# Amanda-Zheng/MR-GNAS

Hardware: AMD Instinct MI355X
Metric: million edges/sec per supernet fwd+bwd step (FB15k-237, dim=200) (higher is better)
Workload: dtype f32

## Files before the change

include/mrgnas.h:

```cpp
#ifndef MRGNAS_H
#define MRGNAS_H

#include <stdint.h>

#ifdef __cplusplus
extern "C" {
#endif

#define MRG_ABI_VERSION 21

#define MRG_OK            0
#define MRG_E_NULLPTR    -1
#define MRG_E_SHAPE      -2
#define MRG_E_ENUM       -3
#define MRG_E_WORKSPACE  -4

#define MRG_COMPOSE_MULT 0
#define MRG_COMPOSE_SUB  1
#define MRG_COMPOSE_ADD  2
#define MRG_REDUCE_SUM   0
#define MRG_REDUCE_MEAN  1
#define MRG_REDUCE_MAX   2
#define MRG_GCS_SUB      0
#define MRG_GCS_MUL      1
#define MRG_GCS_COPY     2
#define MRG_GCS_NEGS     3
#define MRG_GCS_CCORR    4
#define MRG_GCS_CCONV    5
#define MRG_ACT_NONE     0
#define MRG_ACT_RELU     1
#define MRG_ACT_SIGMOID  2

int mrg_abi_version(void);
const char *mrg_error_string(int code);
const char *mrg_target_arch(void);

int mrg_compose_fwd(int op, const float *s, const float *hr, float *out,
                    int64_t rows, int D, void *stream);
int mrg_compose_bwd(int op, const float *gout, const float *s, const float *hr,
                    float *gs, float *ghr, int64_t rows, int D, void *stream);

int mrg_gather_compose_fwd(int op, const float *ent, const float *rel,
                           const int32_t *ent_idx, const int32_t *rel_idx,
                           float *out, int64_t rows, int D, void *stream);

#define MRG_GATE_LD(D) (2 * (D) + 4)

int mrg_gate_collapse3(const float *const *W_host, const float *const *b_host, const float *const *a_host, float *uvc,
                       int D, int in_dim, int fold, void *stream);
int mrg_gate_param_grad3(const float *const *W_host, const float *const *b_host, const float *const *a_host,
                         const float *d_uvc, float *const *gW_host, float *const *gb_host, float *const *ga_host,
                         int D, int in_dim, int fold, void *stream);
int mrg_fold_halves3(const float *const *W_host, float *Wt, int D, void *stream);
int mrg_unfold_halves3(const float *const *gWt_host, float *const *gW_host, int D, void *stream);

int mrg_gate_fwd(const float *s, const float *s_in, const float *norm, const float *uvc,
                 float *out, int64_t b0, int64_t b1, int64_t M, int D, float scale, void *stream);
int64_t mrg_gate_bwd_workspace_bytes(int64_t M, int D);
int mrg_gate_bwd(const float *gout, const float *s, const float *s_in, const float *norm,
                 const float *uvc, float *gs, float *gs_in, float *d_uvc, void *ws,
                 int64_t b0, int64_t b1, int64_t M, int D, float scale, void *stream);
int mrg_gate_row_fwd(const float *s, const float *s_in, const float *norm, const float *uvc, float *fvec, float *hvec,
                     int64_t b0, int64_t b1, int64_t M, int D, float scale, void *stream);
int64_t mrg_gate_row_colsum_blocks(int64_t b0, int64_t b1, int64_t M, int D, int vec4);
int mrg_gate_row_fwd_colsum(const float *s, const float *s_in, const float *norm, const float *uvc, float *fvec, float *hvec,
                            int64_t b0, int64_t b1, int64_t M, int D, float scale, void *stream, double *colsum, int64_t colsum_blocks);
int mrg_gate_row_bwd(const float *q, const float *hvec, const float *s, const float *s_in, const float *uvc, float *gs_in, float *d_uvc,
                     void *ws, int64_t b0, int64_t b1, int64_t M, int D, void *stream);

int64_t mrg_seg_reduce_workspace_bytes(int64_t n_slots, int D);
int mrg_seg_reduce_fwd(int mode, const float *msg, const float *self_rows,
                       const int32_t *eid,
                       const int32_t *chunk_node, const int32_t *chunk_start, const int32_t *chunk_end,
                       const int32_t *chunk_slot, int64_t n_chunks,
                       const int32_t *hub_node, const int32_t *hub_first, const int32_t *hub_count, int64_t n_hubs,
                       int64_t n_slots, const int32_t *in_degree,
                       float *out, int32_t *arg, void *ws,
                       int64_t N, int D, void *stream);
int mrg_seg_reduce_bwd(int mode, const float *gout, const int32_t *dst, const int32_t *in_degree,
                       const int32_t *arg, float *gmsg, float *gself, const float *relu_src,
                       int64_t E, int64_t N, int D, void *stream);
int mrg_seg_reduce_bwd_ordered(int mode, const float *gout, const int32_t *dst, const int32_t *in_degree, const int32_t *arg,
                               float *gmsg, float *gself, const float *relu_src, const unsigned *relu_bits, const int32_t *order,
                               int64_t E, int64_t N, int D, void *stream);
int mrg_segmax_bwd_input_ok(int D, int Kin);
int mrg_segmax_bwd_input(const float *gout, const float *mx, const int32_t *dst, const int32_t *arg, const float *W, float *gmsg,
                         float *gx, const int32_t *order, int64_t E, int64_t N, int D, int Kin, void *stream);

int64_t mrg_seg_std_workspace_bytes(int64_t n_slots, int D);
int mrg_seg_std_fwd(const float *msg, const int32_t *eid, const int32_t *chunk_node, const int32_t *chunk_start,
                    const int32_t *chunk_end, const int32_t *chunk_slot, int64_t n_chunks, const int32_t *hub_node,
                    const int32_t *hub_first, const int32_t *hub_count, int64_t n_hubs, int64_t n_slots,
                    const int32_t *in_degree, float *out, float *mean, float *coef, void *ws, int64_t N, int D, void *stream);
int mrg_seg_std_bwd(const float *gout, const float *msg, const int32_t *dst, const float *mean, const float *coef,
                    const int32_t *order, float *gmsg, int64_t E, int64_t N, int D, void *stream);

int mrg_fused_gcs(int mode, const float *X, const int32_t *xi, const float *Y, const int32_t *yi,
                  const float *scal, const int32_t *eid,
                  const int32_t *chunk_node, const int32_t *chunk_start, const int32_t *chunk_end,
                  const int32_t *chunk_slot, int64_t n_chunks,
                  const int32_t *hub_node, const int32_t *hub_first, const int32_t *hub_count, int64_t n_hubs,
                  int64_t n_slots, const int32_t *seg_len,
                  float *out, void *ws, int64_t nseg, int D, void *stream);

int mrg_span_gcs(int mode, const float *X, const float *Y, const void *meta, const float *ext_scal, int64_t E, int span,
                 const int32_t *span_slot, const int32_t *span_start, int64_t n_spans,
                 const int32_t *hub_seg, const int32_t *hub_first, const int32_t *hub_count, int64_t n_hubs,
                 int64_t n_slots, const int32_t *seg_len,
                 float *out, void *ws, int64_t nseg, int D, void *stream);

int mrg_sum_buffers(const float *const *xs_host, int K, float *out, int64_t n, int accumulate, void *stream);
int mrg_sum_rows_gather(const float *const *xs_host, int K, const float *gather_edge, const float *gather_self,
                        const int32_t *dst, int64_t E, int64_t rows, int D, float *out, void *stream);

int mrg_distmult_score(const float *ent, const float *rel, const int32_t *s_idx, const int32_t *r_idx,
                       const int32_t *o_idx, float *score, int64_t T, int D, void *stream);

int64_t mrg_mix_workspace_bytes(int K, int D);

int mrg_optim_chunk(void);
int mrg_clip_sgd_step(void *const *params, const void *const *grads, void *const *bufs, const int32_t *chunk_tensor,
                      const int64_t *chunk_off, const int32_t *chunk_len, int64_t n_chunks, double *partial, float *norm_coef,
                      float max_norm, float lr, float momentum, float weight_decay, void *stream);
int mrg_adam_step(void *const *params, const void *const *grads, void *const *exp_avg, void *const *exp_avg_sq, int64_t n_tensors,
                  const int32_t *chunk_tensor, const int64_t *chunk_off, const int32_t *chunk_len, int64_t n_chunks, float *step,
                  float *scal, const float *lr, double beta1, double beta2, float eps, float weight_decay, void *stream);
#define MRG_MIX_MAX_CANDIDATES 8
typedef struct mrg_gated_branch {
  int32_t k;
  const float *s;
  const float *rowscale;
  int32_t row_k;
  const float *row_f;
  const float *row_h;
  const float *row_uvc;
  int32_t row_ld;
  int64_t b0, b1;
  float *row_dq;
  int32_t act;
  const int32_t *valid_rows;
// ... 181 lines not shown
```

mr-gnas_amd/_lib.py:

```python
import ctypes
import os
import re

import torch

_HERE = os.path.dirname(os.path.abspath(__file__))
LIB_PATH = os.environ.get("MRG_LIB_PATH") or os.path.join(_HERE, "lib", "libmrgnas_hip.so")
HEADER_PATH = os.path.join(os.path.dirname(_HERE), "include", "mrgnas.h")

ABI_VERSION = 21


class MrgnasLibraryError(RuntimeError):
    pass


class MrgnasError(RuntimeError):
    """A C-ABI call returned a non-zero code."""


_P, _I, _L, _F = ctypes.c_void_p, ctypes.c_int, ctypes.c_int64, ctypes.c_float

SIGNATURES = {
    "mrg_abi_version": (_I, []),
    "mrg_error_string": (ctypes.c_char_p, [_I]),
    "mrg_target_arch": (ctypes.c_char_p, []),
    "mrg_compose_fwd": (_I, [_I, _P, _P, _P, _L, _I, _P]),
    "mrg_compose_bwd": (_I, [_I, _P, _P, _P, _P, _P, _L, _I, _P]),
    "mrg_gather_compose_fwd": (_I, [_I, _P, _P, _P, _P, _P, _L, _I, _P]),
    "mrg_gate_collapse3": (_I, [_P, _P, _P, _P, _I, _I, _I, _P]),
    "mrg_gate_param_grad3": (_I, [_P, _P, _P, _P, _P, _P, _P, _I, _I, _I, _P]),
    "mrg_fold_halves3": (_I, [_P, _P, _I, _P]),
    "mrg_unfold_halves3": (_I, [_P, _P, _I, _P]),
    "mrg_gate_fwd": (_I, [_P, _P, _P, _P, _P, _L, _L, _L, _I, _F, _P]),
    "mrg_gate_bwd_workspace_bytes": (_L, [_L, _I]),
    "mrg_gate_bwd": (_I, [_P, _P, _P, _P, _P, _P, _P, _P, _P, _L, _L, _L, _I, _F, _P]),
    "mrg_seg_reduce_workspace_bytes": (_L, [_L, _I]),
    "mrg_seg_reduce_fwd": (_I, [_I, _P, _P, _P, _P, _P, _P, _P, _L, _P, _P, _P, _L, _L, _P, _P, _P, _P, _L, _I, _P]),
    "mrg_seg_reduce_bwd": (_I, [_I, _P, _P, _P, _P, _P, _P, _P, _L, _L, _I, _P]),
    "mrg_fused_gcs": (_I, [_I, _P, _P, _P, _P, _P, _P, _P, _P, _P, _P, _L, _P, _P, _P, _L, _L, _P, _P, _P, _L, _I, _P]),
    "mrg_span_gcs": (_I, [_I, _P, _P, _P, _P, _L, _I, _P, _P, _L, _P, _P, _P, _L, _L, _P, _P, _P, _L, _I, _P]),
    "mrg_sum_buffers": (_I, [_P, _I, _P, _L, _I, _P]),
    "mrg_sum_rows_gather": (_I, [_P, _I, _P, _P, _P, _L, _L, _I, _P, _P]),
    "mrg_distmult_score": (_I, [_P, _P, _P, _P, _P, _P, _L, _I, _P]),
    "mrg_gate_row_fwd": (_I, [_P, _P, _P, _P, _P, _P, _L, _L, _L, _I, _F, _P]),
    "mrg_gate_row_colsum_blocks": (_L, [_L, _L, _L, _I, _I]),
    "mrg_gate_row_fwd_colsum": (_I, [_P, _P, _P, _P, _P, _P, _L, _L, _L, _I, _F, _P, _P, _L]),
    "mrg_gate_row_bwd": (_I, [_P, _P, _P, _P, _P, _P, _P, _P, _L, _L, _L, _I, _P]),
    "mrg_mix_workspace_bytes": (_L, [_I, _I]),
    "mrg_mix_colstats": (_I, [_P, _I, _L, _I, _P, _P, _P, _P]),
    "mrg_mix_finalize_fwd": (_I, [_P, _P, _P, _P, _P, _I, ctypes.c_double, _I, _F, _F, _P, _P]),
    "mrg_mix_stats_coef": (_I, [_P, _P, _P, _P, _P, _I, _L, ctypes.c_double, _I, _F, _F, _P, _P, _P, _P]),
    "mrg_zero_workspace_bytes": (_L, [_I]),
    "mrg_zero_colstats": (_I, [_P, _P, _P, _P, _P, _I, _L, _I, _P, _P, _P]),
    "mrg_zero_stats_coef": (_I, [_P, _P, _P, _P, _P, _I, _P, _P, _P, _P, _L, ctypes.c_double, _I, _F, _F, _P, _P, _P, _P]),
    "mrg_zero_fwd": (_I, [_P, _P, _P, _P, _P, _I, _P, _P, _P, _L, _I, _P, _P]),
    "mrg_zero_bwd_reduce": (_I, [_P, _P, _P, _P, _P, _P, _I, _P, _P, _P, _P, _L, _I, _P, _P]),
    "mrg_zero_bwd_apply": (_I, [_P, _P, _P, _P, _P, _P, _I, _P, _P, _P, _P, _P, _L, _I, _P, _P]),
    "mrg_mix_fwd": (_I, [_P, _I, _P, _P, _P, _P, _L, _I, _P, _P]),
    "mrg_mix_bwd_reduce": (_I, [_P, _P, _I, _P, _P, _P, _P, _L, _I, _P, _P]),
    "mrg_mix_finalize_bwd": (_I, [_P, _I, ctypes.c_double, _I, _P, _P, _P, _P, _P, _P]),
    "mrg_mix_bwd_apply": (_I, [_P, _P, _P, _I, _P, _P, _P, _P, _P, _P, _P, _P, _P, _P, _P, _P, _P, _L, _I, _P, _P]),
    "mrg_dense_filter_fwd": (_I, [_I, _P, _P, _P, _P, _P, _F, _P, _P, _P, _L, _I, _P]),
    "mrg_dense_filter_dz": (_I, [_I, _P, _P, _P, _P, _F, _P, _P, _L, _I, _P]),
    "mrg_gemm_workspace_bytes": (_L, [_I, _I]),
    "mrg_gemm_set_mode": (_I, [_I]),
    "mrg_gemm_set_epilogue": (_I, [_I]),
    "mrg_gemm_set_wide8": (_I, [_I]),
    "mrg_gemm_set_q": (_I, [_I]),
    "mrg_gemm_set_small": (_I, [_I]),
    "mrg_segmax_bwd_input_ok": (_I, [_I, _I]),
    "mrg_segmax_bwd_input": (_I, [_P, _P, _P, _P, _P, _P, _P, _P, _L, _L, _I, _I, _P]),
    "mrg_seg_std_workspace_bytes": (_L, [_L, _I]),
    "mrg_seg_std_fwd": (_I, [_P, _P, _P, _P, _P, _P, _L, _P, _P, _P, _L, _L, _P, _P, _P, _P, _P, _L, _I, _P]),
    "mrg_seg_std_bwd": (_I, [_P, _P, _P, _P, _P, _P, _P, _L, _L, _I, _P]),
    "mrg_optim_chunk": (_I, []),
    "mrg_clip_sgd_step": (_I, [_P, _P, _P, _P, _P, _P, _L, _P, _P, _F, _F, _F, _F, _P]),
    "mrg_adam_step": (_I, [_P, _P, _P, _P, _L, _P, _P, _P, _L, _P, _P, _P, ctypes.c_double, ctypes.c_double, _F, _F, _P]),
    "mrg_act_grad_transpose": (_I, [_P, _P, _P, _L, _L, _I, _P]),
    "mrg_wgrad_set_variant": (_I, [_I]),
    "mrg_linear_fwd": (_I, [_P, _P, _P, _P, _P, _L, _I, _I, _I, _P]),
    "mrg_dense_filter3_workspace_bytes": (_L, [_I, _I]),
    "mrg_dense_filter_fwd3": (_I, [_I, _P, _P, _P, _P, _P, _F, _F, _P, _P, _P, _L, _L, _L, _I, _P]),
    "mrg_dense_filter3_colsum_blocks": (_L, [_I, _L, _L, _L, _I, _I]),
    "mrg_dense_filter_fwd3_colsum": (_I, [_I, _P, _P, _P, _P, _P, _F, _F, _P, _P, _P, _L, _L, _L, _I, _P, _P, _L]),
    "mrg_dense_filter_dz3": (_I, [_I, _P, _P, _P, _P, _F, _F, _P, _P, _L, _L, _I, _P]),
    "mrg_linear_bwd_input3_workspace_bytes": (_L, [_I, _I]),
    "mrg_linear_bwd_input3": (_I, [_P, _P, _P, _P, _L, _L, _L, _I, _I, _I, _I, _P]),
    "mrg_linear_bwd_input3_pair_workspace_bytes": (_L, [_I, _I]),
    "mrg_linear_bwd_input3_pair": (_I, [_P, _P, _P, _P, _P, _P, _L, _L, _L, _I, _I, _I, _I, _P]),
    "mrg_linear_bwd_weight3_workspace_bytes": (_L, [_L, _L, _L, _I, _I, _I]),
    "mrg_linear_bwd_weight3": (_I, [_P, _P, _P, _P, _P, _P, _L, _L, _L, _I, _I, _I, _P]),
    "mrg_linear_relu_segsum_fwd": (_I, [_P, _P, _P, _P, _P, _P, _P, _P, _L, _I, _I, _P]),
    "mrg_seg_reduce_heads_fwd": (_I, [_I, _P, _P, _P, _P, _P, _P, _P, _L, _P, _P, _P, _L, _L, _P, _P, _P, _L, _I, _P]),
    "mrg_seg_reduce_bwd_bits": (_I, [_I, _P, _P, _P, _P, _P, _P, _L, _L, _I, _P]),
    "mrg_seg_reduce_bwd_ordered": (_I, [_I, _P, _P, _P, _P, _P, _P, _P, _P, _P, _L, _L, _I, _P]),
    "mrg_linear_relu_segmax_workspace_bytes": (_L, [_L, _I, _I]),
    "mrg_linear_relu_segmax_fwd": (_I, [_P, _P, _P, _P, _P, _P, _P, _P, _P, _P, _L, _L, _I, _I, _P]),
    "mrg_linear_bwd_input_workspace_bytes": (_L, [_I, _I]),
    "mrg_linear_bwd_input": (_I, [_P, _P, _P, _P, _L, _I, _I, _I, _I, _P]),
    "mrg_linear_bwd_weight_workspace_bytes": (_L, [_L, _I, _I]),
    "mrg_linear_bwd_weight": (_I, [_P, _P, _P, _P, _P, _P, _L, _I, _I, _I, _P]),
    "mrg_linear_bwd_weight_share": (_I, [_P, _P, _P, _P, _P, _P, _L, _I, _I, _I, _I, _P]),
    "mrg_build_graph_workspace_bytes": (_L, [_L]),
    "mrg_build_graph": (_I, [_P, _L, _L, _I, _I, _P, _L, _P, _P, _P, _P, _P, _P, _P, _P, _P, _P, _L, _P]),
    "mrg_plan_workspace_bytes": (_L, [_L, _L, _I]),
    "mrg_span_plan_build": (_I, [_P, _L, _L, _I, _I, _P, _P, _P, _P, _P, _P, _P, _P, _P, _P, _L, _P]),
    "mrg_span_meta_pack": (_I, [_P, _P, _P, _P, _P, _I, _P, _L, _P]),
    "mrg_chunk_plan_workspace_bytes": (_L, [_L, _L]),
    "mrg_chunk_plan_build": (_I, [_P, _L, _L, _I, _P, _P, _P, _P, _P, _P, _P, _P, _P, _P, _P, _P, _L, _P]),
    "mrg_negative_sampling": (_I, [_P, _L, _I, _P, _P, _P, _P, _P]),
    "mrg_sample_neighborhood_workspace_bytes": (_L, [_L, _L]),
    "mrg_sample_edge_neighborhood": (_I, [_P, _P, _P, _P, _L, _L, _L, _P, _P, _L, _P, _P, _P, _P, _L, _P]),
    "mrg_relabel_workspace_bytes": (_L, [_L]),
    "mrg_relabel_nodes": (_I, [_P, _P, _L, _L, _P, _P, _P, _P, _P, _L, _P]),
    "mrg_multi_hot_labels": (_I, [_P, _P, _P, _P, _L, _L, _L, _F, _F, _P, _P]),
    "mrg_rank_filtered": (_I, [_P, _P, _P, _L, _L, _P, _P]),
    "mrg_transe_score_fwd": (_I, [_P, _P, _P, _F, _P, _L, _L, _I, _P]),
    "mrg_transe_score_bwd": (_I, [_P, _P, _P, _P, _P, _P, _P, _L, _L, _I, _P]),
    "mrg_ccorr_rows": (_I, [_I, _P, _P, _P, _L, _I, _P]),
    "mrg_ccorr_matrix": (_I, [_I, _P, _P, _I, _P]),
    "mrg_ccorr_matrix_grad": (_I, [_I, _P, _P, _I, _P]),
    "mrg_conve_fc_workspace_bytes": (_L, [_L, _L, _I]),
    "mrg_conve_bwd_workspace_bytes": (_L, [_L, _I, _I, _I]),
    "mrg_conve_bn0_fwd": (_I, [_P, _P, _L, _I, _P, _P, _I, _F, _F, _P, _P]),
# ... 178 lines not shown
```

mr-gnas_amd/csrc/segreduce.hip:

```cpp
#include "segcommon.hpp"

namespace mrg {

__device__ __forceinline__ bool seg_is_head(int j, int list_start) {
  const int q = j & 31;
  const int prev = (q & 3) ? j - 1 : (q >= 8 ? j - 5 : -1);
  return prev < list_start;
}

template <int VEC, int LPR, int KMAX, bool IS_MAX, bool HEADS = false>
__global__ __launch_bounds__(MRG_BLOCK) void seg_chunk_k(const float* __restrict__ msg, const float* __restrict__ self_rows,
                                                         const int32_t* __restrict__ eid, const int32_t* __restrict__ chunk_node,
                                                         const int32_t* __restrict__ chunk_start, const int32_t* __restrict__ chunk_end,
                                                         const int32_t* __restrict__ chunk_slot, int64_t n_chunks,
                                                         const int32_t* __restrict__ in_degree, float* __restrict__ out,
                                                         int32_t* __restrict__ arg, float* __restrict__ ws_val,
                                                         int32_t* __restrict__ ws_arg, int D, int is_mean,
                                                         const int32_t* __restrict__ head_rowptr = nullptr) {
  constexpr int RPB = MRG_BLOCK / LPR;
  constexpr int U = 4;
  const int sl = threadIdx.x % LPR, rw = row_group_of_thread<LPR>();
  const int dv = D / VEC;
  for (int64_t ch = (int64_t)blockIdx.x * RPB + rw; ch < n_chunks; ch += (int64_t)gridDim.x * RPB) {
    const int v = chunk_node[ch];
// ... 108 lines not shown
  const int dv = D >> 2, kv = Kin >> 2;
  const int64_t stride = (int64_t)gridDim.x * WAVES;
  auto edge_at = [&](int64_t p) -> int { const int64_t q = p < E ? p : E - 1; return order ? order[q] : (int)q; };
  const bool lv = lane < dv;
  auto load_row = [&](int64_t v, float4& g4, int4& a4, float4& x4) {
    g4 = make_float4(0.f, 0.f, 0.f, 0.f); a4 = make_int4(-1, -1, -1, -1); x4 = make_float4(1.f, 1.f, 1.f, 1.f);
    if (lv) {
      g4 = *reinterpret_cast<const float4*>(gout + v * D + lane * 4);
      a4 = *reinterpret_cast<const int4*>(arg + v * D + lane * 4);
      if (mx) x4 = *reinterpret_cast<const float4*>(mx + v * D + lane * 4);
    }
  };
  const int64_t first = (int64_t)blockIdx.x * WAVES + wave;
  if (first >= E) return;
  int r0 = __builtin_amdgcn_readfirstlane(edge_at(first));
  int r1 = __builtin_amdgcn_readfirstlane(edge_at(first + stride));
  int64_t v1 = __builtin_amdgcn_readfirstlane(dst[r1]);
  float4 g4, x4; int4 a4;
  load_row((int64_t)__builtin_amdgcn_readfirstlane(dst[r0]), g4, a4, x4);
  for (int64_t pos = first; pos < E; pos += stride) {
    const int r2 = __builtin_amdgcn_readfirstlane(edge_at(pos + 2 * stride));
    const int v2 = dst[r2];
    float4 gn, xn; int4 an;
    load_row(v1, gn, an, xn);
    const int r = r0;
    float m[4];
    m[0] = (a4.x == r && x4.x > 0.f) ? g4.x : 0.f;
    m[1] = (a4.y == r && x4.y > 0.f) ? g4.y : 0.f;
    m[2] = (a4.z == r && x4.z > 0.f) ? g4.z : 0.f;
    m[3] = (a4.w == r && x4.w > 0.f) ? g4.w : 0.f;
    if (lv && gmsg) *reinterpret_cast<float4*>(gmsg + (int64_t)r * D + lane * 4) = make_float4(m[0], m[1], m[2], m[3]);
    float4 acc = make_float4(0.f, 0.f, 0.f, 0.f);
#pragma unroll
    for (int j = 0; j < 4; ++j) {
      unsigned long long live = __ballot(m[j] != 0.f);
      while (live) {
        const int src = __builtin_amdgcn_readfirstlane((int)__builtin_ctzll(live));
        live &= live - 1;
        const float val = __int_as_float(__builtin_amdgcn_readlane(__float_as_int(m[j]), src));
        const int c = src * 4 + j;
        if (lane < kv) {
          const float4 w4 = *reinterpret_cast<const float4*>(wsrc + c * Kin + lane * 4);
          acc.x += val * w4.x; acc.y += val * w4.y; acc.z += val * w4.z; acc.w += val * w4.w;
        }
      }
    }
    if (lane < kv) *reinterpret_cast<float4*>(gx + (int64_t)r * Kin + lane * 4) = acc;
    g4 = gn; a4 = an; x4 = xn;
    r0 = r1; r1 = r2;
    v1 = __builtin_amdgcn_readfirstlane(v2);
  }
}

}

using namespace mrg;

extern "C" int mrg_segmax_bwd_input_ok(int D, int Kin) {
  return (D > 0 && Kin > 0 && D % 4 == 0 && Kin % 4 == 0 && D <= 256 && Kin <= 256 && (size_t)D * Kin * 4 <= 160 * 1024) ? 1 : 0;
}

extern "C" int mrg_segmax_bwd_input(const float* gout, const float* mx, const int32_t* dst, const int32_t* arg, const float* W, float* gmsg,
                                    float* gx, const int32_t* order, int64_t E, int64_t N, int D, int Kin, void* stream) {
  if (E < 0 || N < 0 || E >= ((int64_t)1 << 31)) return MRG_E_SHAPE;
  if (!mrg_segmax_bwd_input_ok(D, Kin)) return MRG_E_SHAPE;
  if (E == 0) return MRG_OK;
  if (!gout || !dst || !arg || !W || !gx) return MRG_E_NULLPTR;
  if (!aligned16(gout) || !aligned16(arg) || !aligned16(W) || !aligned16(gx) || !aligned16(gmsg) || !aligned16(mx)) return MRG_E_SHAPE;
  const size_t lds = (size_t)D * Kin * sizeof(float);
  (void)hipFuncSetAttribute(reinterpret_cast<const void*>(&segmax_bwd_gx_k), hipFuncAttributeMaxDynamicSharedMemorySize, (int)lds);
  int64_t grid = (E + 15) / 16;
  if (grid > 256) grid = 256;
  hipLaunchKernelGGL(segmax_bwd_gx_k, dim3((unsigned)grid), dim3(1024), lds, (hipStream_t)stream, gout, mx, dst, arg, W, gmsg, gx, order, E, D, Kin);
  MRG_LAUNCH_CHECK();
  return MRG_OK;
}

extern "C" int64_t mrg_seg_reduce_workspace_bytes(int64_t n_slots, int D) {
  if (n_slots < 0 || D <= 0) return 0;
  return (n_slots + 1) * (int64_t)D * 8 + 64;
}

static int seg_reduce_fwd_impl(int mode, const float* msg, const float* self_rows, const int32_t* eid,
                               const int32_t* chunk_node, const int32_t* chunk_start, const int32_t* chunk_end,
                               const int32_t* chunk_slot, int64_t n_chunks, const int32_t* hub_node,
                               const int32_t* hub_first, const int32_t* hub_count, int64_t n_hubs, int64_t n_slots,
                               const int32_t* in_degree, float* out, int32_t* arg, void* ws, int64_t N, int D,
                               void* stream, const int32_t* head_rowptr);

extern "C" int mrg_seg_reduce_fwd(int mode, const float* msg, const float* self_rows, const int32_t* eid,
                                  const int32_t* chunk_node, const int32_t* chunk_start, const int32_t* chunk_end,
                                  const int32_t* chunk_slot, int64_t n_chunks, const int32_t* hub_node,
                                  const int32_t* hub_first, const int32_t* hub_count, int64_t n_hubs, int64_t n_slots,
                                  const int32_t* in_degree, float* out, int32_t* arg, void* ws, int64_t N, int D,
                                  void* stream) {
  return seg_reduce_fwd_impl(mode, msg, self_rows, eid, chunk_node, chunk_start, chunk_end, chunk_slot, n_chunks, hub_node, hub_first,
                             hub_count, n_hubs, n_slots, in_degree, out, arg, ws, N, D, stream, nullptr);
}

extern "C" int mrg_seg_reduce_heads_fwd(int mode, const float* part, const float* self_rows, const int32_t* rowptr,
                                        const int32_t* chunk_node, const int32_t* chunk_start, const int32_t* chunk_end,
                                        const int32_t* chunk_slot, int64_t n_chunks, const int32_t* hub_node,
                                        const int32_t* hub_first, const int32_t* hub_count, int64_t n_hubs, int64_t n_slots,
                                        const int32_t* in_degree, float* out, void* ws, int64_t N, int D, void* stream) {
  if (mode != MRG_REDUCE_SUM && mode != MRG_REDUCE_MEAN) return MRG_E_ENUM;
  if (!rowptr) return MRG_E_NULLPTR;
  return seg_reduce_fwd_impl(mode, part, self_rows, nullptr, chunk_node, chunk_start, chunk_end, chunk_slot, n_chunks, hub_node, hub_first,
                             hub_count, n_hubs, n_slots, in_degree, out, nullptr, ws, N, D, stream, rowptr);
}
// ... 93 lines not shown
```

mr-gnas_amd/functional/reducers.py:

```python
import os

import torch

from .. import _lib
from .._lib import call, f32c, ptr, require_hip, stream_of
from . import switches as SW
from ._base import REDUCE, _cnt, _ws, _ws_bytes
from .gcs import span_gcs


def _seg_fwd(mode, msg, self_rows, p, N, D, want_arg=True):
    out = torch.empty(N, D, dtype=torch.float32, device=msg.device)
    arg = torch.empty(N, D, dtype=torch.int32, device=msg.device) if mode == 2 else None
    n_chunks, n_hubs, n_slots = _cnt(p, "chunks"), _cnt(p, "hubs"), _cnt(p, "slots")
    ws = _ws(_ws_bytes("mrg_seg_reduce_workspace_bytes", n_slots, D), msg) if n_slots > 0 else None
    E = int(p["eid"].numel())
    nb = 4 * D * E + 4 * E + 4 * D * N * (1 + (self_rows is not None) + (mode == 2))
    call("mrg_seg_reduce_fwd", (mode, ptr(msg), ptr(self_rows), ptr(p["eid"]), ptr(p["chunk_node"]), ptr(p["chunk_start"]),
                                ptr(p["chunk_end"]), ptr(p["chunk_slot"]), n_chunks, ptr(p["hub_node"]),
                                ptr(p["hub_first"]), ptr(p["hub_count"]), n_hubs, n_slots, ptr(p["in_degree"]),
                                ptr(out), ptr(arg), ptr(ws), N, D, stream_of(msg)), nbytes=nb)
    return out, arg


ORDERED_BWD = os.environ.get("MRG_SEG_BWD_ORDERED", "1") == "1"
ORDERED_BWD_MIN_BYTES = int(os.environ.get("MRG_SEG_BWD_ORDERED_MIN_BYTES", str(128 << 20)))


def _seg_bwd(mode, g, graph, arg, gmsg, gself, relu_src=None, relu_bits=None):
    p = graph.plan()
    E, N, D = graph.num_edges(), graph.number_of_nodes(), g.shape[1]
    nb = 4 * D * E * (1 + (relu_src is not None)) + 4 * E + 4 * D * N * (1 + (gself is not None) + (mode == 2))
    big = 4 * D * N * (2 if mode == 2 else 1) > ORDERED_BWD_MIN_BYTES
    order = p["eid"] if (ORDERED_BWD and g.is_cuda and big) else None
    call("mrg_seg_reduce_bwd_ordered", (mode, ptr(g), ptr(graph.i32("dst")), ptr(p["in_degree"]), ptr(arg), ptr(gmsg), ptr(gself),
                                        ptr(relu_src), ptr(relu_bits), ptr(order), E, N, D, stream_of(g)), nbytes=nb)



def _amax_bwd_sparse(g, mx, arg, W, graph, gy, gx):
    E, N, D = graph.num_edges(), graph.number_of_nodes(), g.shape[1]
    if not (SW.SPARSE_AMAX_BWD and g.is_cuda and _lib.load().mrg_segmax_bwd_input_ok(D, W.shape[1])):
        return False
    p = graph.plan()
    big = 4 * D * N * 3 > ORDERED_BWD_MIN_BYTES
    order = p["eid"] if (ORDERED_BWD and big) else None
    call("mrg_segmax_bwd_input", (ptr(g), ptr(mx), ptr(graph.i32("dst")), ptr(arg), ptr(W), ptr(gy), ptr(gx), ptr(order), E, N, D, W.shape[1],
                                  stream_of(g)), nbytes=4 * E * (D + W.shape[1]) + 4 * E + 12 * N * D)
    return True

class _SegReduce(torch.autograd.Function):
    @staticmethod
    def forward(ctx, mode, msg, self_rows, graph):
        msg, self_rows = f32c(msg), f32c(self_rows)
        require_hip(msg, self_rows)
        if msg.shape[0] != graph.num_edges():
            raise _lib.MrgnasError(f"message rows {msg.shape[0]} != number of edges {graph.num_edges()}")
        if mode != 2 and hasattr(graph, "agg_plan"):
            sp, meta = graph.agg_plan("mean" if mode == 1 else "sum")
            out, arg = span_gcs("copy", msg, None, meta, sp), None
            if self_rows is not None:
                out += self_rows
        else:
            out, arg = _seg_fwd(mode, msg, self_rows, graph.plan(), graph.number_of_nodes(), msg.shape[1])
        ctx.mode, ctx.graph, ctx.has_self = mode, graph, self_rows is not None
        ctx.save_for_backward(*((arg,) if arg is not None else ()))
        return out

    @staticmethod
    def backward(ctx, g):
        g = f32c(g)
        arg = ctx.saved_tensors[0] if ctx.mode == 2 else None
        gmsg = torch.empty(ctx.graph.num_edges(), g.shape[1], dtype=torch.float32, device=g.device)
        _seg_bwd(ctx.mode, g, ctx.graph, arg, gmsg, None)
        return None, gmsg, (g if ctx.has_self else None), None


def seg_reduce(kind, msg, self_rows, graph):
    return _SegReduce.apply(REDUCE[kind], msg, self_rows, graph)


class _AggRows(torch.autograd.Function):

    @staticmethod
    def forward(ctx, mode, x, graph, add_self, keep):
        x = f32c(x)
        require_hip(x, keep)
        E, N, D = graph.num_edges(), graph.number_of_nodes(), x.shape[1]
        if x.shape[0] != E + N:
            raise _lib.MrgnasError(f"expected {E + N} rows (E + N), got {x.shape[0]}")
        if mode != 2 and hasattr(graph, "agg_plan"):
            sp, meta = graph.agg_plan("mean" if mode == 1 else "sum")
            out, arg = span_gcs("copy", x, None, meta, sp), None
            if keep is not None:
                out *= keep
            if add_self:
                out += x[E:]
        else:
            out, arg = _seg_fwd(mode, x, x[E:] if (add_self and keep is None) else None, graph.plan(), N, D)
            if keep is not None:
                out *= keep
                if add_self:
# ... 59 lines not shown
            ctx.mode, ctx.graph, ctx.fused = mode, graph, True
            ctx.save_for_backward(x, W, arg, mx)
            if SW.MASK_TAP is not None:
                SW.MASK_TAP(("a_max", W.data_ptr()), [arg, mx > 0])
            return out
        if (mode == 1 and SW.FUSED_AMEAN and E >= SW.FUSED_AMAX_MIN_ROWS and hasattr(graph, "plan")
                and _fused_agg_ws(N, D) > 0):
            p = graph.plan()
            part = torch.empty(E, D, dtype=torch.float32, device=x.device)
            bits = torch.empty(E, (D + 31) // 32, dtype=torch.int32, device=x.device)
            gws = _ws(_ws_bytes("mrg_gemm_workspace_bytes", D, D), x)
            call("mrg_linear_relu_segsum_fwd", (ptr(x), ptr(W), ptr(b), ptr(p["eid"]), ptr(graph.i32("dst")), ptr(part), ptr(bits), ptr(gws),
                                                E, D, D, st), nbytes=4 * E * D + 8 * E + 4 * D * D, flops=2 * E * D * D)
            out = torch.empty(N, D, dtype=torch.float32, device=x.device)
            n_chunks, n_hubs, n_slots = _cnt(p, "chunks"), _cnt(p, "hubs"), _cnt(p, "slots")
            ws = _ws(_ws_bytes("mrg_seg_reduce_workspace_bytes", n_slots, D), x) if n_slots > 0 else None
            call("mrg_seg_reduce_heads_fwd", (1, ptr(part), ptr(x[E:]), ptr(p["rowptr"]), ptr(p["chunk_node"]), ptr(p["chunk_start"]),
                                              ptr(p["chunk_end"]), ptr(p["chunk_slot"]), n_chunks, ptr(p["hub_node"]), ptr(p["hub_first"]),
                                              ptr(p["hub_count"]), n_hubs, n_slots, ptr(p["in_degree"]), ptr(out), ptr(ws), N, D, st),
                 nbytes=8 * N * D + 4 * E)
            ctx.mode, ctx.graph, ctx.fused = mode, graph, "mean"
            ctx.save_for_backward(x, W, bits)
            if SW.MASK_TAP is not None:
                SW.MASK_TAP(("a_mean", W.data_ptr()), [bits])
            return out
        y = torch.empty(E, D, dtype=torch.float32, device=x.device)
        gws = _ws(_ws_bytes("mrg_gemm_workspace_bytes", D, D), x)
        call("mrg_linear_fwd", (ptr(x), ptr(W), ptr(b), ptr(y), ptr(gws), E, D, D, 1, st),
             nbytes=4 * E * 2 * D + 4 * D * D, flops=2 * E * D * D)
        if mode == 2:
            out, arg = _seg_fwd(2, y, x[E:], graph.plan(), N, D)
        else:
            sp, meta = graph.agg_plan("mean" if mode == 1 else "sum")
            out, arg = span_gcs("copy", y, None, meta, sp), None
            out += x[E:]
        ctx.mode, ctx.graph, ctx.fused = mode, graph, False
        ctx.save_for_backward(x, W, y, *((arg,) if arg is not None else ()))
        return out

    @staticmethod
    def backward(ctx, g):
        graph, mode = ctx.graph, ctx.mode
        g = f32c(g)
        if ctx.fused == "mean":
            x, W, bits = ctx.saved_tensors
        elif ctx.fused:
            x, W, arg, mx = ctx.saved_tensors
        else:
            x, W, y, *rest = ctx.saved_tensors
            arg = rest[0] if rest else None
        E, N, D = graph.num_edges(), graph.number_of_nodes(), x.shape[1]
        st = stream_of(x)
        gx = torch.empty_like(x)
        gy = torch.empty(E, D, dtype=torch.float32, device=x.device)
        if ctx.fused == "mean":
            _seg_bwd(1, g, graph, None, gy, gx[E:], relu_bits=bits)
        elif ctx.fused:
            gx[E:] = g
            have_gx = _amax_bwd_sparse(g, mx, arg, W, graph, gy, gx)
            if not have_gx:
                _seg_bwd(mode, g * (mx > 0), graph, arg, gy, None)
        else:
            _seg_bwd(mode, g, graph, arg, gy, gx[E:], relu_src=y)
        work = dict(nbytes=4 * E * 2 * D + 4 * D * D, flops=2 * E * D * D)
        if not (ctx.fused is True and have_gx):
            wt = _ws(_ws_bytes("mrg_linear_bwd_input_workspace_bytes", D, D), x)
            call("mrg_linear_bwd_input", (ptr(gy), ptr(W), ptr(gx), ptr(wt), E, D, D, D, 0, st), **work)
        gW = torch.empty_like(W)
        gb = torch.empty(D, dtype=torch.float32, device=x.device)
        ws = _ws(_ws_bytes("mrg_linear_bwd_weight_workspace_bytes", E, D, D), x)
        call("mrg_linear_bwd_weight", (ptr(gy), ptr(x), None, ptr(gW), ptr(gb), ptr(ws), E, D, 0, D, st), **work)
        return None, gx, gW, gb, None


def linear_relu_aggregate(kind, x, W, b, graph):
    return _LinReluAgg.apply(REDUCE[kind], x, W, b, graph)


class _LinReluPartial(torch.autograd.Function):

    @staticmethod
    def forward(ctx, mode, x, W, b, graph):
        x, W, b = f32c(x), f32c(W), f32c(b)
        require_hip(x, W, b)
        E, N, D = graph.num_edges(), graph.number_of_nodes(), x.shape[1]
        st = stream_of(x)
        fused_ws = _fused_agg_ws(N, D) if (mode == 2 and SW.FUSED_AMAX and E >= SW.FUSED_AMAX_MIN_ROWS) else 0
        if fused_ws > 0:
            out = torch.empty(N, D, dtype=torch.float32, device=x.device)
            arg = torch.empty(N, D, dtype=torch.int32, device=x.device)
            mx = torch.empty(N, D, dtype=torch.float32, device=x.device)
            call("mrg_linear_relu_segmax_fwd", (ptr(x), ptr(W), ptr(b), ptr(graph.plan()["eid"]), ptr(graph.i32("dst")), None, ptr(out), ptr(arg),
                                                ptr(mx), ptr(_ws(fused_ws, x)), E, N, D, D, st),
                 nbytes=4 * E * D + 8 * E + 4 * D * D + 4 * N * D * 3, flops=2 * E * D * D)
            ctx.mode, ctx.graph, ctx.fused = mode, graph, True
            ctx.save_for_backward(x, W, arg, mx)
            if SW.MASK_TAP is not None:
                SW.MASK_TAP(("a_max", W.data_ptr()), [arg, mx > 0])
            return out, x[E:].clone()
        if (mode != 2 and SW.FUSED_AMEAN and E >= SW.FUSED_AMAX_MIN_ROWS and _fused_agg_ws(N, D) > 0):
            p = graph.plan()
            part = torch.empty(E, D, dtype=torch.float32, device=x.device)
            bits = torch.empty(E, (D + 31) // 32, dtype=torch.int32, device=x.device)
            gws = _ws(_ws_bytes("mrg_gemm_workspace_bytes", D, D), x)
            call("mrg_linear_relu_segsum_fwd", (ptr(x), ptr(W), ptr(b), ptr(p["eid"]), ptr(graph.i32("dst")), ptr(part), ptr(bits), ptr(gws),
                                                E, D, D, st), nbytes=4 * E * D + 8 * E + 4 * D * D, flops=2 * E * D * D)
            out = torch.empty(N, D, dtype=torch.float32, device=x.device)
            n_chunks, n_hubs, n_slots = _cnt(p, "chunks"), _cnt(p, "hubs"), _cnt(p, "slots")
            ws = _ws(_ws_bytes("mrg_seg_reduce_workspace_bytes", n_slots, D), x) if n_slots > 0 else None
            call("mrg_seg_reduce_heads_fwd", (0, ptr(part), None, ptr(p["rowptr"]), ptr(p["chunk_node"]), ptr(p["chunk_start"]),
                                              ptr(p["chunk_end"]), ptr(p["chunk_slot"]), n_chunks, ptr(p["hub_node"]), ptr(p["hub_first"]),
                                              ptr(p["hub_count"]), n_hubs, n_slots, ptr(p["in_degree"]), ptr(out), ptr(ws), N, D, st),
                 nbytes=8 * N * D + 4 * E)
            ctx.mode, ctx.graph, ctx.fused = mode, graph, "sum"
            ctx.save_for_backward(x, W, bits)
            return out, x[E:].clone()
        y = torch.empty(E, D, dtype=torch.float32, device=x.device)
        gws = _ws(_ws_bytes("mrg_gemm_workspace_bytes", D, D), x)
        call("mrg_linear_fwd", (ptr(x), ptr(W), ptr(b), ptr(y), ptr(gws), E, D, D, 1, st),
             nbytes=4 * E * 2 * D + 4 * D * D, flops=2 * E * D * D)
        if mode == 2:
            out, arg = _seg_fwd(2, y, None, graph.plan(), N, D)
        else:
            sp, meta = graph.agg_plan("sum")
            out, arg = span_gcs("copy", y, None, meta, sp), None
        ctx.mode, ctx.graph, ctx.fused = mode, graph, False
        ctx.save_for_backward(x, W, y, *((arg,) if arg is not None else ()))
        return out, x[E:].clone()

    @staticmethod
    def backward(ctx, g, gself):
        if ctx.fused == "sum":
            x, W, bits = ctx.saved_tensors
        elif ctx.fused:
            x, W, arg, mx = ctx.saved_tensors
        else:
            x, W, y, *rest = ctx.saved_tensors
            arg = rest[0] if rest else None
        graph, mode = ctx.graph, ctx.mode
        E, D = graph.num_edges(), x.shape[1]
        g = f32c(g) if g is not None else torch.zeros(graph.number_of_nodes(), D, dtype=torch.float32, device=x.device)
        st = stream_of(x)
        gx = torch.empty_like(x)
        if gself is not None:
            gx[E:] = gself
        else:
            gx[E:].zero_()
        gy = torch.empty(E, D, dtype=torch.float32, device=x.device)
        if ctx.fused == "sum":
            _seg_bwd(0, g, graph, None, gy, None, relu_bits=bits)
        elif ctx.fused:
            have_gx = _amax_bwd_sparse(g, mx, arg, W, graph, gy, gx)
            if not have_gx:
                _seg_bwd(mode, g * (mx > 0), graph, arg, gy, None)
        else:
            _seg_bwd(mode, g, graph, arg, gy, None, relu_src=y)
        work = dict(nbytes=4 * E * 2 * D + 4 * D * D, flops=2 * E * D * D)
        if not (ctx.fused is True and have_gx):
            wt = _ws(_ws_bytes("mrg_linear_bwd_input_workspace_bytes", D, D), x)
            call("mrg_linear_bwd_input", (ptr(gy), ptr(W), ptr(gx), ptr(wt), E, D, D, D, 0, st), **work)
        gW = torch.empty_like(W)
        gb = torch.empty(D, dtype=torch.float32, device=x.device)
        ws = _ws(_ws_bytes("mrg_linear_bwd_weight_workspace_bytes", E, D, D), x)
        call("mrg_linear_bwd_weight", (ptr(gy), ptr(x), None, ptr(gW), ptr(gb), ptr(ws), E, D, 0, D, st), **work)
        return None, gx, gW, gb, None


def linear_relu_partial(kind, x, W, b, graph):
    return _LinReluPartial.apply(REDUCE[kind], x, W, b, graph)


class _SumPartial(torch.autograd.Function):

    @staticmethod
    def forward(ctx, x, graph):
        x = f32c(x)
        require_hip(x)
        E = graph.num_edges()
        sp, meta = graph.agg_plan("sum")
        ctx.graph = graph
        ctx.shape = x.shape
        return span_gcs("copy", x, None, meta, sp), x[E:].clone()

    @staticmethod
    def backward(ctx, g, gself):
        graph = ctx.graph
        E, D = graph.num_edges(), ctx.shape[1]
        gx = torch.empty(ctx.shape, dtype=torch.float32, device=(g if g is not None else gself).device)
        if gself is not None:
            gx[E:] = gself
        else:
            gx[E:].zero_()
        if g is not None:
            _seg_bwd(0, f32c(g), graph, None, gx, None)
        else:
            gx[:E].zero_()
        return gx, None


def sum_partial(x, graph):
    return _SumPartial.apply(x, graph)
```

mr-gnas_amd/functional/switches.py:

```python
import os

ROW_FACTOR = os.environ.get("MRG_ROW_FACTOR", "1") == "1"
LAZY_ASUM = os.environ.get("MRG_LAZY_ASUM", "1") == "1"
FUSED_AMAX = os.environ.get("MRG_FUSED_AMAX", "1") == "1"
FUSED_AMAX_MIN_ROWS = int(os.environ.get("MRG_FUSED_AMAX_MIN_ROWS", "100000"))
FUSED_AMEAN = os.environ.get("MRG_FUSED_AMEAN", "1") == "1"
WIDE_BWD_INPUT = os.environ.get("MRG_WIDE_BWD_INPUT", "1") == "1"
NODE_LINEAR = os.environ.get("MRG_NODE_LINEAR", "1") == "1"
MASK_TAP = None
FOLD_IDENTITY = os.environ.get("MRG_FOLD_IDENTITY", "1") == "1"
CELL_ZERO_FUSED = os.environ.get("MRG_CELL_ZERO_FUSED", "1") == "1"
FORK_MIN_ROWS = int(os.environ.get("MRG_FORK_MIN_ROWS", str(1 << 17)))
SEGMENT_STREAMS = int(os.environ.get("MRG_SEGMENT_STREAMS", "3"))
FOLD_ROW_SCALE = os.environ.get("MRG_FOLD_ROW_SCALE", "1") == "1"
GROUPED_SEGMENTS = os.environ.get("MRG_GROUPED_SEGMENTS", "1") == "1"
DENSE_PAIR = os.environ.get("MRG_DENSE_PAIR", "1") == "1"
GATED_RECOMPUTE = os.environ.get("MRG_GATED_RECOMPUTE", "1") == "1"
PRODUCER_STATS = os.environ.get("MRG_PRODUCER_STATS", "1") == "1"
COMPGCN_TAIL = os.environ.get("MRG_COMPGCN_TAIL", "1") == "1"
SPARSE_AMAX_BWD = os.environ.get("MRG_SPARSE_AMAX_BWD", "1") == "1"
CCORR_PATH = None
```

Baseline: 11.76.

## Compute max-aggregation weight gradient sparsely from argmax winners, skipping dense gy

```diff
diff --git a/include/mrgnas.h b/include/mrgnas.h
--- a/include/mrgnas.h
+++ b/include/mrgnas.h
@@ -7,7 +7,7 @@
 extern "C" {
 #endif
 
-#define MRG_ABI_VERSION 21
+#define MRG_ABI_VERSION 22
 
 #define MRG_OK            0
 #define MRG_E_NULLPTR    -1
@@ -86,6 +86,10 @@
 int mrg_segmax_bwd_input_ok(int D, int Kin);
 int mrg_segmax_bwd_input(const float *gout, const float *mx, const int32_t *dst, const int32_t *arg, const float *W, float *gmsg,
                          float *gx, const int32_t *order, int64_t E, int64_t N, int D, int Kin, void *stream);
+int mrg_segmax_bwd_weight_ok(int D, int K);
+int64_t mrg_segmax_bwd_weight_workspace_bytes(int64_t E, int D, int K);
+int mrg_segmax_bwd_weight(const float *gout, const float *mx, const int32_t *arg, const float *x, const int32_t *eid,
+                          const int32_t *dst, float *gW, float *gb, void *ws, int64_t E, int64_t N, int D, int K, void *stream);
 
 int64_t mrg_seg_std_workspace_bytes(int64_t n_slots, int D);
 int mrg_seg_std_fwd(const float *msg, const int32_t *eid, const int32_t *chunk_node, const int32_t *chunk_start,
diff --git a/mr-gnas_amd/_lib.py b/mr-gnas_amd/_lib.py
--- a/mr-gnas_amd/_lib.py
+++ b/mr-gnas_amd/_lib.py
@@ -8,7 +8,7 @@
 LIB_PATH = os.environ.get("MRG_LIB_PATH") or os.path.join(_HERE, "lib", "libmrgnas_hip.so")
 HEADER_PATH = os.path.join(os.path.dirname(_HERE), "include", "mrgnas.h")
 
-ABI_VERSION = 21
+ABI_VERSION = 22
 
 
 class MrgnasLibraryError(RuntimeError):
@@ -71,6 +71,9 @@
     "mrg_gemm_set_small": (_I, [_I]),
     "mrg_segmax_bwd_input_ok": (_I, [_I, _I]),
     "mrg_segmax_bwd_input": (_I, [_P, _P, _P, _P, _P, _P, _P, _P, _L, _L, _I, _I, _P]),
+    "mrg_segmax_bwd_weight_ok": (_I, [_I, _I]),
+    "mrg_segmax_bwd_weight_workspace_bytes": (_L, [_L, _I, _I]),
+    "mrg_segmax_bwd_weight": (_I, [_P, _P, _P, _P, _P, _P, _P, _P, _P, _L, _L, _I, _I, _P]),
     "mrg_seg_std_workspace_bytes": (_L, [_L, _I]),
     "mrg_seg_std_fwd": (_I, [_P, _P, _P, _P, _P, _P, _L, _P, _P, _P, _L, _L, _P, _P, _P, _P, _P, _L, _I, _P]),
     "mrg_seg_std_bwd": (_I, [_P, _P, _P, _P, _P, _P, _P, _L, _L, _I, _P]),
diff --git a/mr-gnas_amd/csrc/segreduce.hip b/mr-gnas_amd/csrc/segreduce.hip
--- a/mr-gnas_amd/csrc/segreduce.hip
+++ b/mr-gnas_amd/csrc/segreduce.hip
@@ -184,9 +184,214 @@
   }
 }
 
+constexpr int SBW_WAVES = 16, SBW_SUM_WAVES = 13, SBW_ROWS = 64;
+template <int QPW>
+__global__ __launch_bounds__(1024) void segmax_bwd_weight_k(const float* __restrict__ gout, const float* __restrict__ mx,
+                                                          const int32_t* __restrict__ arg, const float* __restrict__ x,
+                                                          const int32_t* __restrict__ eid, const int32_t* __restrict__ dst,
+                                                          float* __restrict__ part, int64_t E, int D, int K, int q0, int q1) {
+  extern __shared__ __align__(16) float xs[];
+  constexpr int CW = SBW_SUM_WAVES, LW = SBW_WAVES - CW, ROWS = SBW_ROWS, XT = (ROWS + LW - 1) / LW;
+  const int tid = threadIdx.x, lane = tid & 63, wave = __builtin_amdgcn_readfirstlane(tid >> 6);
+  const int kv = K >> 2, dq = q1;
+  const int n_stages = (int)((E + ROWS - 1) / ROWS), G = gridDim.x;
+  auto lane_id = [&](int s) -> int { const int64_t pos = (int64_t)s * ROWS + lane; return pos < E ? eid[pos] : -1; };
+  const int s0 = blockIdx.x;
+  int ej = lane_id(s0), ej_nxt = lane_id(s0 + G);
+
+  if (wave >= CW) {
+    const int l = wave - CW;
+    auto issue = [&](int e, float4 (&r)[XT]) {
+#pragma unroll
+      for (int t = 0; t < XT; ++t) {
+        const int row = min(l + t * LW, ROWS - 1);
+        const int et = max(__shfl(e, row), 0);
+        r[t] = make_float4(0.f, 0.f, 0.f, 0.f);
+        if (lane < kv) r[t] = *reinterpret_cast<const float4*>(x + (int64_t)et * K + lane * 4);
+      }
+    };
+    auto commit = [&](float* buf, const float4 (&r)[XT]) {
+#pragma unroll
+      for (int t = 0; t < XT; ++t) {
+        const int row = min(l + t * LW, ROWS - 1);
+        if (lane < kv) *reinterpret_cast<float4*>(buf + row * K + lane * 4) = r[t];
+      }
+    };
+    float4 r[XT];
+    issue(ej, r);
+    commit(xs, r);
+    issue(ej_nxt, r);
+    __syncthreads();
+    int buf = 0;
+    for (int s = s0; s < n_stages; s += G) {
+      const int ej_nn = lane_id(s + 2 * G);
+      if (s + G < n_stages) commit(xs + (buf ^ 1) * ROWS * K, r);
+      issue(ej_nn, r);
+      __syncthreads();
+      buf ^= 1;
+    }
+    return;
+  }
+
+  float4 acc[QPW * 4];
+#pragma unroll
+  for (int i = 0; i < QPW * 4; ++i) acc[i] = make_float4(0.f, 0.f, 0.f, 0.f);
+  float gbv[QPW];
+#pragma unroll
+  for (int q = 0; q < QPW; ++q) gbv[q] = 0.f;
+
+  auto heads = [&](int e, int d, bool& hd, int& hl) {
+    const int prev = __shfl_up(d, 1);
+    hd = e >= 0 && (lane == 0 || d != prev);
+    const unsigned long long hb = __ballot(hd);
+    hl = e >= 0 ? 63 - __builtin_clzll(hb & (~0ull >> (63 - lane))) : 0;
+  };
+  auto load_q = [&](int q, bool hd, int d, int4& a4, float4& g4, float4& x4) {
+    a4 = make_int4(-1, -1, -1, -1); g4 = make_float4(0.f, 0.f, 0.f, 0.f); x4 = make_float4(1.f, 1.f, 1.f, 1.f);
+    const int cq = q0 + wave + CW * q;
+    if (cq < dq && hd) {
+      const int64_t off = (int64_t)d * D + cq * 4;
+      a4 = *reinterpret_cast<const int4*>(arg + off);
+      g4 = *reinterpret_cast<const float4*>(gout + off);
+      if (mx) x4 = *reinterpret_cast<const float4*>(mx + off);
+    }
+  };
+  int dj = ej >= 0 ? dst[ej] : -1;
+  bool head; int hl;
+  heads(ej, dj, head, hl);
+  constexpr int AH = QPW < 4 ? QPW : 2;
+  int4 ta[QPW]; float4 tg[QPW], tx[QPW];
+#pragma unroll
+  for (int q = 0; q < AH; ++q) load_q(q, head, dj, ta[q], tg[q], tx[q]);
+  __syncthreads();
+  int buf = 0;
+  for (int s = s0; s < n_stages; s += G) {
+    const int dj_nxt = ej_nxt >= 0 ? dst[ej_nxt] : -1;
+    const int ej_nn = lane_id(s + 2 * G);
+    const float* __restrict__ xb = xs + buf * ROWS * K;
+    float tm[QPW][4];
+#pragma unroll
+    for (int q = AH; q < QPW; ++q) load_q(q, head, dj, ta[q], tg[q], tx[q]);
+#pragma unroll
+    for (int q = 0; q < AH; ++q) {
+      tm[q][0] = tx[q].x > 0.f ? tg[q].x : 0.f; tm[q][1] = tx[q].y > 0.f ? tg[q].y : 0.f;
+      tm[q][2] = tx[q].z > 0.f ? tg[q].z : 0.f; tm[q][3] = tx[q].w > 0.f ? tg[q].w : 0.f;
+    }
+#pragma unroll
+    for (int q = 0; q < QPW; ++q) {
+      if (q >= AH) {
+        tm[q][0] = tx[q].x > 0.f ? tg[q].x : 0.f; tm[q][1] = tx[q].y > 0.f ? tg[q].y : 0.f;
+        tm[q][2] = tx[q].z > 0.f ? tg[q].z : 0.f; tm[q][3] = tx[q].w > 0.f ? tg[q].w : 0.f;
+      }
+      if (q0 + wave + CW * q < dq) {
+        const int a[4] = {ta[q].x, ta[q].y, ta[q].z, ta[q].w};
+        const float* m = tm[q];
+#pragma unroll
+        for (int i = 0; i < 4; ++i) {
+          const int ah = __shfl(a[i], hl);
+          const float mh = __shfl(m[i], hl);
+          const float v = (ej >= 0 && ah == ej) ? mh : 0.f;
+          unsigned long long live = __ballot(v != 0.f);
+          while (live) {
+            const int j = __builtin_amdgcn_readfirstlane((int)__builtin_ctzll(live));
+            live &= live - 1;
+            const float val = __int_as_float(__builtin_amdgcn_readlane(__float_as_int(v), j));
+            if (lane < kv) {
+              const float4 r = *reinterpret_cast<const float4*>(xb + j * K + lane * 4);
+              float4& o = acc[q * 4 + i];
+              o.x += val * r.x; o.y += val * r.y; o.z += val * r.z; o.w += val * r.w;
+            }
+            if (lane == i) gbv[q] += val;
+          }
+        }
+      }
+    }
+    ej = ej_nxt; dj = dj_nxt; ej_nxt = ej_nn;
+    heads(ej, dj, head, hl);
+#pragma unroll
+    for (int q = 0; q < AH; ++q) load_q(q, head, dj, ta[q], tg[q], tx[q]);
+    __syncthreads();
+    buf ^= 1;
+  }
+
+  float* __restrict__ o = part + (int64_t)blockIdx.x * ((int64_t)D * K + D);
+#pragma unroll
+  for (int q = 0; q < QPW; ++q) {
+    const int cq = q0 + wave + CW * q;
+    if (cq < dq && lane < kv) {
+#pragma unroll
+      for (int i = 0; i < 4; ++i) *reinterpret_cast<float4*>(o + (int64_t)(cq * 4 + i) * K + lane * 4) = acc[q * 4 + i];
+    }
+    if (cq < dq && lane < 4) o[(int64_t)D * K + cq * 4 + lane] = gbv[q];
+  }
+}
+
+__global__ void segmax_bwd_weight_reduce_k(const float* __restrict__ ws, float* __restrict__ gW, float* __restrict__ gb, int nb, int lenW, int D) {
+  __shared__ double part[16][64];
+  const int tx = threadIdx.x & 63, ty = threadIdx.x >> 6;
+  const int t = blockIdx.x * 64 + tx, ld = lenW + D;
+  part[ty][tx] = t < ld ? ordered_partial<float>(ws, 0, nb, ld, t, ty) : 0.0;
+  __syncthreads();
+  if (ty == 0 && t < ld) {
+    double tot = part[0][tx];
+#pragma unroll
+    for (int i = 1; i < 16; ++i) tot += part[i][tx];
+    if (t < lenW) gW[t] = (float)tot;
+    else if (gb) gb[t - lenW] = (float)tot;
+  }
+}
+
 }
 
 using namespace mrg;
+
+extern "C" int mrg_segmax_bwd_weight_ok(int D, int K) {
+  return (D > 0 && K > 0 && D % 4 == 0 && K % 4 == 0 && D <= 256 && K <= 256) ? 1 : 0;
+}
+
+static int segmax_bwd_weight_grid(int64_t E) {
+  const int64_t stages = (E + 63) / 64;
+  return (int)(stages < 256 ? stages : 256);
+}
+
+extern "C" int64_t mrg_segmax_bwd_weight_workspace_bytes(int64_t E, int D, int K) {
+  if (E <= 0 || E >= ((int64_t)1 << 31) || !mrg_segmax_bwd_weight_ok(D, K)) return 0;
+  return (int64_t)segmax_bwd_weight_grid(E) * ((int64_t)D * K + D) * (int64_t)sizeof(float);
+}
+
+extern "C" int mrg_segmax_bwd_weight(const float* gout, const float* mx, const int32_t* arg, const float* x, const int32_t* eid,
+                                     const int32_t* dst, float* gW, float* gb, void* ws, int64_t E, int64_t N, int D, int K, void* stream) {
+  if (E < 0 || N < 0 || E >= ((int64_t)1 << 31)) return MRG_E_SHAPE;
+  if (!mrg_segmax_bwd_weight_ok(D, K)) return MRG_E_SHAPE;
+  if (!gW) return MRG_E_NULLPTR;
+  hipStream_t st = (hipStream_t)stream;
+  if (E == 0) {
+    hipError_t e = hipMemsetAsync(gW, 0, sizeof(float) * (size_t)D * K, st);
+    if (e == hipSuccess && gb) e = hipMemsetAsync(gb, 0, sizeof(float) * (size_t)D, st);
+    return (int)e;
+  }
+  if (!gout || !arg || !x || !eid || !dst) return MRG_E_NULLPTR;
+  if (!ws) return MRG_E_WORKSPACE;
+  if (!aligned16(gout) || !aligned16(mx) || !aligned16(arg) || !aligned16(x) || !aligned16(ws)) return MRG_E_SHAPE;
+  const int grid = segmax_bwd_weight_grid(E), dq = D / 4;
+  const size_t lds = (size_t)2 * SBW_ROWS * K * sizeof(float);
+  const int n_launch = dq > 4 * SBW_SUM_WAVES ? 2 : 1;
+  for (int h = 0; h < n_launch; ++h) {
+    const int q0 = h * (dq / n_launch), q1 = h + 1 == n_launch ? dq : (h + 1) * (dq / n_launch);
+    const int qpw = (q1 - q0 + SBW_SUM_WAVES - 1) / SBW_SUM_WAVES;
+#define CALL(Q)                                                                                                        \
+  do {                                                                                                                 \
+    (void)hipFuncSetAttribute(reinterpret_cast<const void*>(&segmax_bwd_weight_k<Q>), hipFuncAttributeMaxDynamicSharedMemorySize, (int)lds); \
+    hipLaunchKernelGGL((segmax_bwd_weight_k<Q>), dim3(grid), dim3(1024), lds, st, gout, mx, arg, x, eid, dst, (float*)ws, E, D, K, q0, q1); \
+  } while (0)
+    if (qpw == 1) CALL(1); else if (qpw == 2) CALL(2); else if (qpw == 3) CALL(3); else CALL(4);
+#undef CALL
+    MRG_LAUNCH_CHECK();
+  }
+  hipLaunchKernelGGL(segmax_bwd_weight_reduce_k, dim3((D * K + D + 63) / 64), dim3(1024), 0, st, (const float*)ws, gW, gb, grid, D * K, D);
+  MRG_LAUNCH_CHECK();
+  return MRG_OK;
+}
 
 extern "C" int mrg_segmax_bwd_input_ok(int D, int Kin) {
   return (D > 0 && Kin > 0 && D % 4 == 0 && Kin % 4 == 0 && D <= 256 && Kin <= 256 && (size_t)D * Kin * 4 <= 160 * 1024) ? 1 : 0;
diff --git a/mr-gnas_amd/functional/reducers.py b/mr-gnas_amd/functional/reducers.py
--- a/mr-gnas_amd/functional/reducers.py
+++ b/mr-gnas_amd/functional/reducers.py
@@ -38,16 +38,28 @@
 
 
 
-def _amax_bwd_sparse(g, mx, arg, W, graph, gy, gx):
-    E, N, D = graph.num_edges(), graph.number_of_nodes(), g.shape[1]
-    if not (SW.SPARSE_AMAX_BWD and g.is_cuda and _lib.load().mrg_segmax_bwd_input_ok(D, W.shape[1])):
-        return False
+def _amax_bwd_sparse(g, mx, arg, W, x, graph, gx):
+    E, N, D, K = graph.num_edges(), graph.number_of_nodes(), g.shape[1], W.shape[1]
+    lib = _lib.load()
+    if not (SW.SPARSE_AMAX_BWD and g.is_cuda and lib.mrg_segmax_bwd_input_ok(D, K)):
+        return False, None, None, None
     p = graph.plan()
+    sparse_w = bool(SW.SPARSE_AMAX_WGRAD and E >= SW.SPARSE_AMAX_WGRAD_MIN_ROWS and lib.mrg_segmax_bwd_weight_ok(D, K))
+    gy = None if sparse_w else torch.empty(E, D, dtype=torch.float32, device=g.device)
     big = 4 * D * N * 3 > ORDERED_BWD_MIN_BYTES
     order = p["eid"] if (ORDERED_BWD and big) else None
-    call("mrg_segmax_bwd_input", (ptr(g), ptr(mx), ptr(graph.i32("dst")), ptr(arg), ptr(W), ptr(gy), ptr(gx), ptr(order), E, N, D, W.shape[1],
-                                  stream_of(g)), nbytes=4 * E * (D + W.shape[1]) + 4 * E + 12 * N * D)
-    return True
+    dst = graph.i32("dst")
+    call("mrg_segmax_bwd_input", (ptr(g), ptr(mx), ptr(dst), ptr(arg), ptr(W), ptr(gy), ptr(gx), ptr(order), E, N, D, K,
+                                  stream_of(g)), nbytes=4 * E * ((0 if sparse_w else D) + K) + 4 * E + 12 * N * D)
+    if not sparse_w:
+        return True, gy, None, None
+    gW = torch.empty_like(W)
+    gb = torch.empty(D, dtype=torch.float32, device=g.device)
+    ws = _ws(_ws_bytes("mrg_segmax_bwd_weight_workspace_bytes", E, D, K), g)
+    call("mrg_segmax_bwd_input", (ptr(g), ptr(mx), ptr(arg), ptr(x), ptr(p["eid"]), ptr(dst), ptr(gW), ptr(gb), ptr(ws), E, N, D, K,
+                                  stream_of(g)), symbol="mrg_segmax_bwd_weight", nbytes=4 * E * K + 4 * E + 12 * N * D + 4 * D * K)
+    return True, None, gW, gb
+
 
 class _SegReduce(torch.autograd.Function):
     @staticmethod
@@ -213,24 +225,29 @@
         E, N, D = graph.num_edges(), graph.number_of_nodes(), x.shape[1]
         st = stream_of(x)
         gx = torch.empty_like(x)
-        gy = torch.empty(E, D, dtype=torch.float32, device=x.device)
+        new_gy = lambda: torch.empty(E, D, dtype=torch.float32, device=x.device)
+        gW = gb = None
         if ctx.fused == "mean":
+            gy = new_gy()
             _seg_bwd(1, g, graph, None, gy, gx[E:], relu_bits=bits)
         elif ctx.fused:
             gx[E:] = g
-            have_gx = _amax_bwd_sparse(g, mx, arg, W, graph, gy, gx)
+            have_gx, gy, gW, gb = _amax_bwd_sparse(g, mx, arg, W, x, graph, gx)
             if not have_gx:
+                gy = new_gy()
                 _seg_bwd(mode, g * (mx > 0), graph, arg, gy, None)
         else:
+            gy = new_gy()
             _seg_bwd(mode, g, graph, arg, gy, gx[E:], relu_src=y)
         work = dict(nbytes=4 * E * 2 * D + 4 * D * D, flops=2 * E * D * D)
         if not (ctx.fused is True and have_gx):
             wt = _ws(_ws_bytes("mrg_linear_bwd_input_workspace_bytes", D, D), x)
             call("mrg_linear_bwd_input", (ptr(gy), ptr(W), ptr(gx), ptr(wt), E, D, D, D, 0, st), **work)
-        gW = torch.empty_like(W)
-        gb = torch.empty(D, dtype=torch.float32, device=x.device)
-        ws = _ws(_ws_bytes("mrg_linear_bwd_weight_workspace_bytes", E, D, D), x)
-        call("mrg_linear_bwd_weight", (ptr(gy), ptr(x), None, ptr(gW), ptr(gb), ptr(ws), E, D, 0, D, st), **work)
+        if gW is None:
+            gW = torch.empty_like(W)
+            gb = torch.empty(D, dtype=torch.float32, device=x.device)
+            ws = _ws(_ws_bytes("mrg_linear_bwd_weight_workspace_bytes", E, D, D), x)
+            call("mrg_linear_bwd_weight", (ptr(gy), ptr(x), None, ptr(gW), ptr(gb), ptr(ws), E, D, 0, D, st), **work)
         return None, gx, gW, gb, None
 
 
@@ -307,23 +324,28 @@
             gx[E:] = gself
         else:
             gx[E:].zero_()
-        gy = torch.empty(E, D, dtype=torch.float32, device=x.device)
+        new_gy = lambda: torch.empty(E, D, dtype=torch.float32, device=x.device)
+        gW = gb = None
         if ctx.fused == "sum":
+            gy = new_gy()
             _seg_bwd(0, g, graph, None, gy, None, relu_bits=bits)
         elif ctx.fused:
-            have_gx = _amax_bwd_sparse(g, mx, arg, W, graph, gy, gx)
+            have_gx, gy, gW, gb = _amax_bwd_sparse(g, mx, arg, W, x, graph, gx)
             if not have_gx:
+                gy = new_gy()
                 _seg_bwd(mode, g * (mx > 0), graph, arg, gy, None)
         else:
+            gy = new_gy()
             _seg_bwd(mode, g, graph, arg, gy, None, relu_src=y)
         work = dict(nbytes=4 * E * 2 * D + 4 * D * D, flops=2 * E * D * D)
         if not (ctx.fused is True and have_gx):
             wt = _ws(_ws_bytes("mrg_linear_bwd_input_workspace_bytes", D, D), x)
             call("mrg_linear_bwd_input", (ptr(gy), ptr(W), ptr(gx), ptr(wt), E, D, D, D, 0, st), **work)
-        gW = torch.empty_like(W)
-        gb = torch.empty(D, dtype=torch.float32, device=x.device)
-        ws = _ws(_ws_bytes("mrg_linear_bwd_weight_workspace_bytes", E, D, D), x)
-        call("mrg_linear_bwd_weight", (ptr(gy), ptr(x), None, ptr(gW), ptr(gb), ptr(ws), E, D, 0, D, st), **work)
+        if gW is None:
+            gW = torch.empty_like(W)
+            gb = torch.empty(D, dtype=torch.float32, device=x.device)
+            ws = _ws(_ws_bytes("mrg_linear_bwd_weight_workspace_bytes", E, D, D), x)
+            call("mrg_linear_bwd_weight", (ptr(gy), ptr(x), None, ptr(gW), ptr(gb), ptr(ws), E, D, 0, D, st), **work)
         return None, gx, gW, gb, None
 
 
diff --git a/mr-gnas_amd/functional/switches.py b/mr-gnas_amd/functional/switches.py
--- a/mr-gnas_amd/functional/switches.py
+++ b/mr-gnas_amd/functional/switches.py
@@ -19,4 +19,6 @@
 PRODUCER_STATS = os.environ.get("MRG_PRODUCER_STATS", "1") == "1"
 COMPGCN_TAIL = os.environ.get("MRG_COMPGCN_TAIL", "1") == "1"
 SPARSE_AMAX_BWD = os.environ.get("MRG_SPARSE_AMAX_BWD", "1") == "1"
+SPARSE_AMAX_WGRAD = os.environ.get("MRG_SPARSE_AMAX_WGRAD", "1") == "1"
+SPARSE_AMAX_WGRAD_MIN_ROWS = int(os.environ.get("MRG_SPARSE_AMAX_WGRAD_MIN_ROWS", "100000"))
 CCORR_PATH = None
```

Result: no change. 11.79 (median of 6 runs) (+0.3%).
